# libav/libav

Hardware: AMD Instinct MI355X
Metric: macroblocks_per_s (higher is better)
Workload: dtype u8

## Files before the change

### include/mi355_h264_frame.h

```cpp
#ifndef MI355_H264_FRAME_H
#define MI355_H264_FRAME_H

#include <stddef.h>
#include <stdint.h>

#ifdef __cplusplus
extern "C" {
#endif

#define MI355_MB_INTRA4x4    0x00000001u
#define MI355_MB_INTRA16x16  0x00000002u
#define MI355_MB_INTRA_PCM   0x00000004u
#define MI355_MB_16x16       0x00000008u
#define MI355_MB_16x8        0x00000010u
#define MI355_MB_8x16        0x00000020u
#define MI355_MB_8x8         0x00000040u
#define MI355_MB_P0L0        0x00001000u
#define MI355_MB_P1L0        0x00002000u
#define MI355_MB_P0L1        0x00004000u
#define MI355_MB_P1L1        0x00008000u
#define MI355_MB_8x8DCT      0x01000000u
#define MI355_MB_INTRA       (MI355_MB_INTRA4x4 | MI355_MB_INTRA16x16 | MI355_MB_INTRA_PCM)

#define MI355_MBF_LEFT_EDGE  0x01
// ... 58 lines not shown
#define MI355_H264_MAX_SLOTS 32

typedef struct mi355_h264_slice {
    uint8_t use_weight;
    uint8_t use_weight_chroma;
    uint8_t luma_log2_weight_denom;
    uint8_t chroma_log2_weight_denom;
    uint8_t list_count;
    uint8_t reserved[3];
    uint8_t ref_slot[2][MI355_H264_MAX_REFS];
    int16_t luma_weight[MI355_H264_MAX_REFS][2][2];
    int16_t chroma_weight[MI355_H264_MAX_REFS][2][2][2];
    int16_t implicit_weight[MI355_H264_MAX_REFS][MI355_H264_MAX_REFS];
    uint8_t chroma_qp_table[2][52];
    int16_t implicit_weight_field[2][2 * MI355_H264_MAX_REFS][2 * MI355_H264_MAX_REFS];
} mi355_h264_slice;

typedef struct mi355_h264_frame {
    int32_t mb_width, mb_height;
    uint8_t *dst[3];
    int32_t dst_stride[2];
    uint8_t *recon[3];
    int32_t recon_stride[2];
    const uint8_t *ref[MI355_H264_MAX_SLOTS][3];
    const mi355_h264_mb *mb;
    const int16_t *mv[2];
    const int16_t *coef;
    const mi355_h264_slice *slices;
    int32_t nslices;
    int32_t max_intra_level;
    const uint32_t *intra_list;
    const int32_t *intra_level_start;
    int32_t max_level_width;
    int32_t field_picture;
    int32_t surface_layout;
    int32_t flags;
} mi355_h264_frame;
#define MI355_FRAME_NO_INTER 1
#define MI355_FRAME_MBAFF    2

#define MI355_SURFACE_LINEAR 0
#define MI355_SURFACE_TILED  1
#define MI355_LAYOUTS_LINEAR 1
#define MI355_LAYOUTS_TILED  2
#define MI355_TILE_LUMA_BYTES   256
#define MI355_TILE_CHROMA_BYTES 128

typedef struct mi355_surface_job {
    uint8_t *lin[3];
    uint8_t *tiled[2];
    int32_t lin_stride[2];
    int32_t tiled_stride[2];
    int32_t mb_width, mb_height;
    int32_t to_tiled;
    int32_t reserved0;
} mi355_surface_job;
int mi355_h264_surface_convert_dev(const mi355_surface_job *jobs, int n, int max_mb_width, int max_mb_height, void *stream);

int mi355_h264_decode_frames(const mi355_h264_frame *frames, int nframes, void *stream);

int mi355_h264_decode_frames_dev(const mi355_h264_frame *d_frames, int nframes,
                                 int max_mb_width, int max_mb_height, int max_intra_level,
                                 int max_level_width, void *stream);

int mi355_h264_decode_frames_levels_dev(const mi355_h264_frame *d_frames, int nframes,
                                        int max_mb_width, int max_mb_height, int max_intra_level,
                                        const int32_t *level_widths, void *stream);

int mi355_h264_decode_frames_layouts_dev(const mi355_h264_frame *d_frames, int nframes,
                                         int max_mb_width, int max_mb_height, int max_intra_level,
                                         const int32_t *level_widths, int layouts, void *stream);

int mi355_h264_decode_frames_wide_dev(const mi355_h264_frame *d_frames, int nframes, int max_mb_width, int max_mb_height,
                                      int max_intra_level, const int32_t *level_widths, int bit_depth, int chroma_format_idc,
                                      int passes, void *stream);

int mi355_h264_recon_intra_levels_dev(const mi355_h264_frame *d_frames, int nframes, int max_intra_level, const int32_t *level_widths, void *stream);
int mi355_h264_recon_intra_all_dev(const mi355_h264_frame *d_frames, int nframes, int max_mb_width, int max_mb_height, int max_intra_level, const int32_t *level_widths, void *stream);
int mi355_h264_recon_intra_plan(int max_mb_width, int max_mb_height, int max_intra_level, const int32_t *level_widths, int pinned, int *single, long long *per_picture);
int mi355_h264_recon_inter_dev(const mi355_h264_frame *d_frames, int nframes, int max_mb_width, int max_mb_height, void *stream);
int mi355_h264_recon_inter_layouts_dev(const mi355_h264_frame *d_frames, int nframes, int max_mb_width, int max_mb_height, int layouts, void *stream);
int mi355_h264_recon_run_plan(int nframes, int max_mb_width, int max_mb_height, int forced, int *run, int *runs_row);
int mi355_h264_recon_inter_run_dev(const mi355_h264_frame *d_frames, int nframes, int max_mb_width, int max_mb_height, int run, void *stream);
int mi355_h264_recon_inter_sparse_dev(const mi355_h264_frame *d_frames, int nframes, int max_mb_width, int max_mb_height, void *stream);
int mi355_h264_recon_intra_dev(const mi355_h264_frame *d_frames, int nframes, int max_intra_level, int max_level_width, void *stream);
int mi355_h264_deblock_dev(const mi355_h264_frame *d_frames, int nframes, int max_mb_width, int max_mb_height, void *stream);
int mi355_h264_deblock_layouts_dev(const mi355_h264_frame *d_frames, int nframes, int max_mb_width, int max_mb_height, int layouts, void *stream);
int mi355_h264_deblock_resident_dev(const mi355_h264_frame *d_frames, int nframes, int max_mb_width, int max_mb_height, int layouts,
                                    int resident_waves, void *stream);
int mi355_h264_deblock_resident(int nframes, int max_mb_width, int max_mb_height, int layouts, int cus, int shares, int *resident_waves);

typedef struct mi355_h264_deblock_plan_info {
    int32_t tiled_waves;
    int32_t linear_bands;
    int32_t skip_tiled;
    int32_t linear_launches;
} mi355_h264_deblock_plan_info;
int mi355_h264_deblock_plan(int nframes, int max_mb_width, int max_mb_height, int layouts, int cus, mi355_h264_deblock_plan_info *plan);
int mi355_h264_deblock_form_dev(const mi355_h264_frame *d_frames, int nframes, int max_mb_width, int max_mb_height, int layouts,
                                int tiled_waves, int linear_bands, void *stream);

int mi355_h264_intra_schedule(mi355_h264_mb *mb, int mb_width, int mb_height,
                              uint32_t *list, int32_t *level_start, int *max_level_width);

int mi355_h264_intra_schedule_mbaff(mi355_h264_mb *mb, int mb_width, int mb_height,
                                    uint32_t *list, int32_t *level_start, int *max_level_width);

void *mi355_malloc(size_t bytes);
void  mi355_free(void *dptr);
int   mi355_memcpy_h2d(void *dst, const void *src, size_t bytes);
int   mi355_memcpy_d2h(void *dst, const void *src, size_t bytes);
int   mi355_memcpy_d2d(void *dst, const void *src, size_t bytes);
int   mi355_sync(void *stream);
void  mi355_prefer_blocking_sync(int on);
void *mi355_host_alloc(size_t bytes);
void  mi355_host_free(void *p);
int   mi355_memcpy_h2d_async(void *dst, const void *src, size_t bytes, void *stream);
int   mi355_memcpy_d2h_async(void *dst, const void *src, size_t bytes, void *stream);
int   mi355_memcpy2d_d2h_async(void *dst, size_t dst_pitch, const void *src, size_t src_pitch, size_t width_bytes, size_t rows, void *stream);
int   mi355_memcpy2d_d2d_async(void *dst, size_t dst_pitch, const void *src, size_t src_pitch, size_t width_bytes, size_t rows, void *stream);
int   mi355_event_sync(void *event);
typedef struct mi355_copy_job {
    const void *src;
    void *dst;
    uint64_t bytes;
} mi355_copy_job;
int   mi355_copy_batch_dev(const mi355_copy_job *jobs, int n, size_t max_bytes, void *stream);
typedef struct mi355_h264_pipelines mi355_h264_pipelines;
mi355_h264_pipelines *mi355_h264_pipelines_create(int shares, int turns);
void mi355_h264_pipelines_destroy(mi355_h264_pipelines *p);
int  mi355_h264_pipelines_decode_dev(mi355_h264_pipelines *p, const mi355_h264_frame *d_frames, int nframes, int max_mb_width, int max_mb_height,
                                     int max_intra_level, const int32_t *level_widths, int layouts);
int  mi355_h264_pipelines_sync(mi355_h264_pipelines *p);
int  mi355_h264_pipelines_share(const mi355_h264_pipelines *p, int nframes, int share, int *first, int *count);
void mi355_h264_pipelines_timing(mi355_h264_pipelines *p, int on);
void mi355_h264_pipelines_join(mi355_h264_pipelines *p, int mode);
int  mi355_h264_pipelines_collect(mi355_h264_pipelines *p, double sums[3], int *launches);

void *mi355_stream_create(void);
void  mi355_stream_destroy(void *stream);
int   mi355_stream_wait_event(void *stream, void *event);
void *mi355_event_create(void);
void  mi355_event_destroy(void *event);
int   mi355_event_record(void *event, void *stream);
int   mi355_event_query(void *event);
float mi355_event_elapsed_ms(void *start, void *end);

#ifdef __cplusplus
}
#endif
#endif
```

### libav_amd/csrc/h264_frame.hip

```cpp
#include <cstdlib>
#include <vector>
#include "h264_recon_dev.h"
#include "../../include/mi355dsp.h"


namespace {

__attribute__((amdgpu_waves_per_eu(MI355_RECON_WAVES, MI355_RECON_WAVES)))
__global__ void __launch_bounds__(64)
k_recon_inter(const mi355_h264_frame *__restrict__ frames, int max_w, int max_h, unsigned long long inv_w, unsigned long long inv_h, int nblocks, int per_xcd)
{
    __shared__ MbLds s;
    recon_inter_wave<false>(s, frames, max_w, max_h, inv_w, inv_h, nblocks, per_xcd);
}
__attribute__((amdgpu_waves_per_eu(MI355_RECON_WAVES, MI355_RECON_WAVES)))
__global__ void __launch_bounds__(64)
k_recon_inter_sparse(const mi355_h264_frame *__restrict__ frames, int max_w, int max_h, unsigned long long inv_w, unsigned long long inv_h, int nblocks, int per_xcd)
{
    __shared__ MbLds s;
    recon_inter_wave<true>(s, frames, max_w, max_h, inv_w, inv_h, nblocks, per_xcd);
}

constexpr int TP = 32;
constexpr int CP = 16;
// ... 133 lines not shown
            MI355_WAVE_SYNC();
        }
    } else {
        for (int i = 0; i < 16; i++) {
            const int x0 = 4 * blk_x4(i), y0 = 4 * blk_y4(i);
            const int tr_ok = (h.topright_samples_available << i) & 0x8000;
            if (lane < 5) s.ps.T[lane] = TILE(x0 + lane - 1, y0 - 1);
            else if (lane < 9) s.ps.T[lane] = tr_ok ? TILE(x0 + lane - 1, y0 - 1) : TILE(x0 + 3, y0 - 1);
            if (lane >= 32 && lane < 37) s.ps.L[lane - 32] = TILE(x0 - 1, y0 + lane - 33);
            MI355_WAVE_SYNC();
            intra_pred_wave(s.ps, 0, h.u.intra4x4_pred_mode[i], 0, 0, &TILE(x0, y0), TP);
            const int q = lane & 3;
            int c[4], r[4], row;
#pragma unroll
            for (int k2 = 0; k2 < 4; k2++) c[k2] = s.mb.coef[i * 16 + q + 4 * k2];
            idct4_quad(c, q, r, row);
            if (lane < 4 && ((h.nnz_mask >> i) & 1)) add_row4<true>(&TILE(x0, y0 + row), r);
            MI355_WAVE_SYNC();
        }
    }
    if (!(t & MI355_MB_INTRA16x16)) residual_chroma<true>(s.mb, &CTILE(0, 0, 0), &CTILE(1, 0, 0), CP);
    intra_store_mb<TILED, AGENT>(&TILE(0, 0), TP, &CTILE(0, 0, 0), &CTILE(1, 0, 0), CP, fr, mb_x, mb_y);
}
#undef TILE

__global__ void __launch_bounds__(64)
k_recon_intra(const mi355_h264_frame *frames, int level, int width)
{
    __shared__ IntraLds s;
    const int f = blockIdx.x / width, k = blockIdx.x - f * width;
    const mi355_h264_frame &frd = frames[f];
    if (level > frd.max_intra_level) return;
    const int first = mi355_global(frd.intra_level_start)[level - 1], count = mi355_global(frd.intra_level_start)[level] - first;
    if (k >= count) return;
    const int mb_xy = (int)mi355_global(frd.intra_list)[first + k];
    if (uniform(frd.surface_layout) == MI355_SURFACE_TILED) recon_intra_mb<true>(s, frd, mb_xy);
    else recon_intra_mb<false>(s, frd, mb_xy);
}

constexpr int INTRA_SINGLE_LEVELS = 16;
constexpr uint32_t INTRA_NAPS_MAX = 1u << 21;
#ifdef MI355_HIP_EMU_H
static inline uint32_t intra_flag_word(const uint8_t *p) { uint32_t v; std::memcpy(&v, reinterpret_cast<const uint8_t *>(reinterpret_cast<uintptr_t>(p) & ~(uintptr_t)3), 4); return v; }
static inline void intra_flag_set(uint8_t *p) { *p = 1; }
#else
__device__ __forceinline__ uint32_t intra_flag_word(const uint8_t *p) { return agent_load_u32(reinterpret_cast<const uint32_t *>(reinterpret_cast<uintptr_t>(p) & ~(uintptr_t)3)); }
__device__ __forceinline__ void intra_flag_set(uint8_t *p) { __hip_atomic_store(p, (uint8_t)1, __ATOMIC_RELAXED, __HIP_MEMORY_SCOPE_AGENT); }
#endif
__global__ void __launch_bounds__(64)
k_recon_intra_all(const mi355_h264_frame *__restrict__ frames, int nframes, int nmb_max, uint8_t *__restrict__ flags, uint32_t *error_word, uint32_t naps_max)
{
    __shared__ IntraLds s;
    const int k = (int)(blockIdx.x / (unsigned)nframes), f = (int)(blockIdx.x - (unsigned)k * (unsigned)nframes);
    const mi355_h264_frame &frd = frames[f];
    const int nlev = uniform(frd.max_intra_level);
    if (nlev <= 0) return;
    if (k >= uniform(mi355_global(frd.intra_level_start)[nlev])) return;
    const int mb_xy = (int)uniform((int)mi355_global(frd.intra_list)[k]);
    const int W = uniform(frd.mb_width), mb_y = mb_xy / W, mb_x = mb_xy - mb_y * W;
    uint8_t *const pic_flags = mi355_global(flags) + (size_t)f * (size_t)nmb_max;
    const int lane = lane_id();
    const int nx = mb_x + (lane == 3 ? 1 : (lane == 2 ? 0 : -1)), ny = mb_y - (lane == 0 ? 0 : 1);
    const bool inside = lane < 4 && nx >= 0 && nx < W && ny >= 0;
    const int nxy = inside ? ny * W + nx : mb_xy;
    const bool dep = inside && (mi355_global_v(reinterpret_cast<const uint32_t *>(mi355_global(frd.mb) + nxy))[0] & MI355_MB_INTRA) != 0;
    static_assert(offsetof(mi355_h264_mb, mb_type) == 0, "the type word of a record");
    const bool waits = __any(dep);
    if (waits) {
        const uint8_t *fp = pic_flags + nxy;
        const int sh = 8 * (int)(reinterpret_cast<uintptr_t>(fp) & 3);
        uint32_t naps = 0;
        while (__any(dep && ((intra_flag_word(fp) >> sh) & 0xFFu) == 0) && naps < naps_max) { wave_nap(); naps++; }
        if (naps >= naps_max && __any(dep && ((intra_flag_word(fp) >> sh) & 0xFFu) == 0) && lane_id() == 0) atomicOr(error_word, (uint32_t)MI355_ERR_WAIT_EXPIRED);
        MI355_ISSUE_FENCE();
    }
    if (uniform(frd.surface_layout) == MI355_SURFACE_TILED) recon_intra_mb<true, true>(s, frd, mb_xy, waits);
    else recon_intra_mb<false, true>(s, frd, mb_xy, waits);
    agent_drain_stores();
    if (lane == 0 && naps_max) intra_flag_set(pic_flags + mb_xy);
}

}

static int recon_inter_launch(const mi355_h264_frame *d_frames, int nframes, int max_mb_width, int max_mb_height, bool sparse, void *stream, int layouts = MI355_LAYOUTS_LINEAR | MI355_LAYOUTS_TILED, int tiled_run = 0)
{
    if (!mi355::bind() || !d_frames || nframes <= 0) return -1;
    const int per_frame = max_mb_width * max_mb_height;
    if (per_frame <= 0 || per_frame >= (1 << 24)) return -3;
    const int frames_per_launch = ((1 << 24) - 1) / per_frame;
    const unsigned long long one = 1ull << 40;
    for (int f0 = 0; f0 < nframes; f0 += frames_per_launch) {
        const int nf = nframes - f0 < frames_per_launch ? nframes - f0 : frames_per_launch;
        const int nblocks = nf * per_frame, per_xcd = (nblocks + 7) / 8;
        const unsigned long long iw = (one + max_mb_width - 1) / max_mb_width, ih = (one + max_mb_height - 1) / max_mb_height;
        if (sparse)
            hipLaunchKernelGGL(k_recon_inter_sparse, dim3((unsigned)(8 * per_xcd)), dim3(64), 0, (hipStream_t)stream,
                               d_frames + f0, max_mb_width, max_mb_height, iw, ih, nblocks, per_xcd);
        else if (layouts == MI355_LAYOUTS_TILED) {
            if (!mi355::recon_inter_tiled_launch(d_frames + f0, nf, max_mb_width, max_mb_height, (hipStream_t)stream, tiled_run)) return -4;
        }
        else
            hipLaunchKernelGGL(k_recon_inter, dim3((unsigned)(8 * per_xcd)), dim3(64), 0, (hipStream_t)stream,
                               d_frames + f0, max_mb_width, max_mb_height, iw, ih, nblocks, per_xcd);
    }
    return hipGetLastError() == hipSuccess ? 0 : -2;
}
extern "C" int mi355_h264_recon_inter_dev(const mi355_h264_frame *d_frames, int nframes, int max_mb_width, int max_mb_height, void *stream)
{
    return recon_inter_launch(d_frames, nframes, max_mb_width, max_mb_height, false, stream);
}
extern "C" int mi355_h264_recon_inter_layouts_dev(const mi355_h264_frame *d_frames, int nframes, int max_mb_width, int max_mb_height, int layouts, void *stream)
{
    if (!(layouts & (MI355_LAYOUTS_LINEAR | MI355_LAYOUTS_TILED))) return -1;
    return recon_inter_launch(d_frames, nframes, max_mb_width, max_mb_height, false, stream, layouts);
}
extern "C" int mi355_h264_recon_inter_run_dev(const mi355_h264_frame *d_frames, int nframes, int max_mb_width, int max_mb_height, int run, void *stream)
{
    int r, runs_row;
    if (run <= 0 || !mi355::recon_run_plan(nframes, max_mb_width, max_mb_height, run, &r, &runs_row)) return -1;
    return recon_inter_launch(d_frames, nframes, max_mb_width, max_mb_height, false, stream, MI355_LAYOUTS_TILED, run);
}
extern "C" int mi355_h264_recon_inter_sparse_dev(const mi355_h264_frame *d_frames, int nframes, int max_mb_width, int max_mb_height, void *stream)
{
    return recon_inter_launch(d_frames, nframes, max_mb_width, max_mb_height, true, stream);
}

extern "C" int mi355_h264_recon_intra_dev(const mi355_h264_frame *d_frames, int nframes, int max_intra_level, int max_level_width, void *stream)
{
    if (!mi355::bind() || !d_frames || nframes <= 0) return -1;
    if (max_intra_level <= 0 || max_level_width <= 0) return 0;
    for (int level = 1; level <= max_intra_level; level++)
        hipLaunchKernelGGL(k_recon_intra, dim3((unsigned)(nframes * max_level_width)), dim3(64), 0, (hipStream_t)stream,
                           d_frames, level, max_level_width);
    return hipGetLastError() == hipSuccess ? 0 : -2;
}

static bool recon_intra_plan(int max_mb_width, int max_mb_height, int max_intra_level, const int32_t *level_widths, int pinned, long long *per_picture)
{
    *per_picture = 0;
    if (pinned == 0 || (pinned != 1 && max_intra_level < INTRA_SINGLE_LEVELS)) return false;
    long long sum = 0;
    for (int level = 1; level <= max_intra_level; level++) sum += level_widths[level - 1] > 0 ? level_widths[level - 1] : 0;
    const long long nmb = (long long)max_mb_width * max_mb_height;
    *per_picture = sum > nmb ? nmb : sum;
    return true;
}
static int intra_single_pin()
{
    static const int single = std::getenv("MI355_INTRA_SINGLE") ? std::atoi(std::getenv("MI355_INTRA_SINGLE")) : -1;
    return single;
}
extern "C" int mi355_h264_recon_intra_plan(int max_mb_width, int max_mb_height, int max_intra_level, const int32_t *level_widths, int pinned, int *single, long long *per_picture)
{
    if (max_mb_width <= 0 || max_mb_height <= 0 || max_intra_level < 0 || (max_intra_level > 0 && !level_widths) || !single || !per_picture) return -1;
    *single = recon_intra_plan(max_mb_width, max_mb_height, max_intra_level, level_widths, pinned < 0 ? intra_single_pin() : pinned, per_picture) ? 1 : 0;
    return 0;
}

extern "C" int mi355_h264_recon_intra_all_dev(const mi355_h264_frame *d_frames, int nframes, int max_mb_width, int max_mb_height, int max_intra_level, const int32_t *level_widths, void *stream)
{
    if (!mi355::bind() || !d_frames || nframes <= 0 || max_mb_width <= 0 || max_mb_height <= 0 || (max_intra_level > 0 && !level_widths)) return -1;
    long long per_picture = 0;
    if (!recon_intra_plan(max_mb_width, max_mb_height, max_intra_level, level_widths, intra_single_pin(), &per_picture))
        return mi355_h264_recon_intra_levels_dev(d_frames, nframes, max_intra_level, level_widths, stream);
    if (per_picture <= 0) return 0;
    const long long nmb = (long long)max_mb_width * max_mb_height;
    if ((long long)nframes * per_picture > 0x7FFFFFFFLL || (long long)nframes * nmb > 0x7FFFFFFFLL) return -3;
    const size_t bytes = ((size_t)nframes * (size_t)nmb + 3) & ~(size_t)3;
    uint32_t *flags = mi355::sync_words((hipStream_t)stream, bytes / 4);
    if (!flags) return -4;
    MI355_TRY(hipMemsetAsync(flags, 0, bytes, (hipStream_t)stream), -4);
    uint32_t *err = mi355::error_word();
    if (!err) return -4;
    static const uint32_t naps_max = std::getenv("MI355_INTRA_NAPS_MAX") ? (uint32_t)std::strtoul(std::getenv("MI355_INTRA_NAPS_MAX"), nullptr, 0) : INTRA_NAPS_MAX;
    hipLaunchKernelGGL(k_recon_intra_all, dim3((unsigned)(nframes * per_picture)), dim3(64), 0, (hipStream_t)stream, d_frames, nframes, (int)nmb, reinterpret_cast<uint8_t *>(flags), err, naps_max);
    return hipGetLastError() == hipSuccess ? 0 : -2;
}

extern "C" int mi355_h264_recon_intra_levels_dev(const mi355_h264_frame *d_frames, int nframes, int max_intra_level, const int32_t *level_widths, void *stream)
{
    if (!mi355::bind() || !d_frames || nframes <= 0 || (max_intra_level > 0 && !level_widths)) return -1;
    for (int level = 1; level <= max_intra_level; level++) {
        const int width = level_widths[level - 1];
        if (width <= 0) continue;
        if ((long long)nframes * width > 0x7FFFFFFFLL) return -3;
        hipLaunchKernelGGL(k_recon_intra, dim3((unsigned)(nframes * width)), dim3(64), 0, (hipStream_t)stream, d_frames, level, width);
    }
    return hipGetLastError() == hipSuccess ? 0 : -2;
}

#ifdef MI355_PROF
extern "C" void mi355_debug_rprof(unsigned long long *out, int reset)
{
    unsigned long long z[16] = {};
    MI355_CHECK(hipDeviceSynchronize());
    MI355_CHECK(hipMemcpyFromSymbol(out, HIP_SYMBOL(g_rprof), sizeof(z)));
    if (reset) MI355_CHECK(hipMemcpyToSymbol(HIP_SYMBOL(g_rprof), z, sizeof(z)));
}
#endif

extern "C" int mi355_h264_decode_frames_dev(const mi355_h264_frame *d_frames, int nframes, int max_mb_width, int max_mb_height,
                                            int max_intra_level, int max_level_width, void *stream)
{
// ... 279 lines not shown
```

### libav_amd/csrc/h264_frame_dev.h

```cpp
#ifndef MI355_H264_FRAME_DEV_H
#define MI355_H264_FRAME_DEV_H

#include "mi355_rt.h"
#include "h264_dev.h"
#include "../../include/mi355_h264_frame.h"

namespace mi355 {

typedef uint32_t mi355_u32x4 __attribute__((vector_size(16)));
typedef uint32_t mi355_u32x2 __attribute__((vector_size(8)));
typedef uint32_t mi355_u32x4u __attribute__((vector_size(16), aligned(4)));
typedef uint32_t mi355_u32x2u __attribute__((vector_size(8), aligned(4)));

__device__ __forceinline__ int blk_x4(int i) { return (i & 1) + 2 * ((i >> 2) & 1); }
__device__ __forceinline__ int blk_y4(int i) { return ((i >> 1) & 1) + 2 * (i >> 3); }
__device__ __forceinline__ int blk_index(int x4, int y4) { return (x4 & 1) + 2 * (y4 & 1) + 4 * (x4 >> 1) + 8 * (y4 >> 1); }

__device__ __forceinline__ uint32_t tile_y_off(int mb_x, int mb_y, int stride) { return (uint32_t)(__mul24(mb_y, stride) + mb_x * MI355_TILE_LUMA_BYTES); }
__device__ __forceinline__ uint32_t tile_c_off(int mb_x, int mb_y, int stride) { return (uint32_t)(__mul24(mb_y, stride) + mb_x * MI355_TILE_CHROMA_BYTES); }

__device__ __forceinline__ uint4 lds16(const uint8_t *p)
{
    const uint2 a = reinterpret_cast<const uint2 *>(p)[0], b = reinterpret_cast<const uint2 *>(p)[1];
    return make_uint4(a.x, a.y, b.x, b.y);
}
__device__ __forceinline__ void lds16(uint8_t *p, uint4 v)
{
    reinterpret_cast<mi355_u32x2 *>(p)[0] = mi355_u32x2{ v.x, v.y };
    reinterpret_cast<mi355_u32x2 *>(p)[1] = mi355_u32x2{ v.z, v.w };
}
__device__ __forceinline__ uint4 ld16(const uint8_t *p, bool al)
{
    if (al) return *reinterpret_cast<const uint4 *>(p);
    const uint32_t *w = reinterpret_cast<const uint32_t *>(p);
    return make_uint4(w[0], w[1], w[2], w[3]);
}
__device__ __forceinline__ void st16(uint8_t *p, uint4 v, bool al)
{
    if (al) { *reinterpret_cast<mi355_u32x4 *>(p) = mi355_u32x4{ v.x, v.y, v.z, v.w }; return; }
    uint32_t *w = reinterpret_cast<uint32_t *>(p);
    w[0] = v.x; w[1] = v.y; w[2] = v.z; w[3] = v.w;
}
__device__ __forceinline__ uint2 ld8(const uint8_t *p, bool al)
{
    if (al) return *reinterpret_cast<const uint2 *>(p);
    const uint32_t *w = reinterpret_cast<const uint32_t *>(p);
    return make_uint2(w[0], w[1]);
}
__device__ __forceinline__ void st8(uint8_t *p, uint2 v, bool al)
{
    if (al) { *reinterpret_cast<mi355_u32x2 *>(p) = mi355_u32x2{ v.x, v.y }; return; }
    uint32_t *w = reinterpret_cast<uint32_t *>(p);
    w[0] = v.x; w[1] = v.y;
}

bool recon_run_plan(int nframes, int max_w, int max_h, int forced, int *run, int *runs_row);
bool recon_inter_tiled_launch(const mi355_h264_frame *d_frames, int nframes, int max_w, int max_h, hipStream_t stream, int forced_run = 0);
void recon_inter_rest_launch(const mi355_h264_frame *d_frames, int max_w, int max_h, int run, int runs_row, unsigned long long inv_runs, unsigned long long inv_h, int nruns,
                             const uint32_t *rest, hipStream_t stream);
uint32_t *sync_words(hipStream_t stream, size_t words);
}
namespace {
#ifdef MI355_HIP_EMU_H
static inline uint32_t agent_load_u32(const uint32_t *p) { return *p; }
static inline void agent_store_u32(uint32_t *p, uint32_t v) { *p = v; }
static inline void agent_store8(uint8_t *p, uint2 v, bool al8) { mi355::st8(p, v, al8); }
static inline void agent_drain_stores() {}
static inline void wave_nap() { std::fprintf(stderr, "k_deblock_tiled: a band waits for a band that has not run (emulator: workgroups run in order)\n"); std::abort(); }
#else
__device__ __forceinline__ uint32_t agent_load_u32(const uint32_t *p) { return __hip_atomic_load(p, __ATOMIC_RELAXED, __HIP_MEMORY_SCOPE_AGENT); }
__device__ __forceinline__ void agent_store_u32(uint32_t *p, uint32_t v) { __hip_atomic_store(p, v, __ATOMIC_RELAXED, __HIP_MEMORY_SCOPE_AGENT); }
__device__ __forceinline__ void agent_store8(uint8_t *p, uint2 v, bool al8)
{
    if (al8) { __hip_atomic_store(reinterpret_cast<unsigned long long *>(p), (unsigned long long)v.x | ((unsigned long long)v.y << 32), __ATOMIC_RELAXED, __HIP_MEMORY_SCOPE_AGENT); return; }
    uint32_t *w = reinterpret_cast<uint32_t *>(p);
    agent_store_u32(w, v.x); agent_store_u32(w + 1, v.y);
}
__device__ __forceinline__ void agent_drain_stores() { asm volatile("s_waitcnt vmcnt(0)" ::: "memory"); }
__device__ __forceinline__ void wave_nap() { __builtin_amdgcn_s_sleep(16); }
#endif
}
#ifdef MI355_HIP_EMU_H
template <bool AGENT> static inline void lds_dma16(const uint8_t *src, uint8_t *lds_base) { std::memcpy(lds_base + 16 * (threadIdx.x & 63), src, 16); }
#else
template <bool AGENT> __device__ __forceinline__ void lds_dma16(const uint8_t *src, uint8_t *lds_base)
{
    typedef __attribute__((address_space(1))) const void *gptr;
    typedef __attribute__((address_space(3))) void *lptr;
    __builtin_amdgcn_global_load_lds((gptr)src, (lptr)lds_base, 16, 0, AGENT ? 16 : 0);
}
#endif
#ifdef MI355_HIP_EMU_H
static inline void lds_dma_wait() {}
#else
__device__ __forceinline__ void lds_dma_wait() { asm volatile("s_waitcnt vmcnt(0)" ::: "memory"); }
#endif

#endif
```

### libav_amd/csrc/h264_frame_tiled.hip

```cpp
#define MI355_PLAIN_LANE 1
#include "h264_recon_fast.h"

#include <cstdlib>

namespace {
__attribute__((amdgpu_waves_per_eu(MI355_RECON_WAVES, MI355_RECON_WAVES)))
__global__ void __launch_bounds__(64)
k_recon_inter_tiled(const mi355_h264_frame *__restrict__ frames, int max_w, int max_h, int run, int runs_row, unsigned long long inv_runs, unsigned long long inv_h, int nwaves, int per_xcd,
                    uint32_t *__restrict__ rest)
{
    __shared__ MbLds s;
    recon_inter_run(s, frames, max_w, max_h, run, runs_row, inv_runs, inv_h, nwaves, per_xcd, rest);
}
}

namespace mi355 {
bool recon_run_plan(int nframes, int max_w, int max_h, int forced, int *run_out, int *runs_row_out)
{
    if (nframes <= 0 || max_w <= 0 || max_h <= 0 || forced < 0) return false;
    const long long mbs = (long long)nframes * max_w * max_h;
    int run = (int)(mbs / (40ll * 8192));
    run = forced > 0 ? forced : (run < 4 ? 4 : (run > 15 ? 15 : run));
    if (run > max_w) run = max_w;
    const int runs_row = (max_w + run - 1) / run;
    run = (max_w + runs_row - 1) / runs_row;
    if (run > 16) return false;
    *run_out = run;
    *runs_row_out = runs_row;
    return true;
}

bool recon_inter_tiled_launch(const mi355_h264_frame *d_frames, int nframes, int max_w, int max_h, hipStream_t stream, int forced_run)
{
    static const int env = std::getenv("MI355_RECON_RUN") ? std::atoi(std::getenv("MI355_RECON_RUN")) : 0;
    static const int forced = env > 0 ? (env < 4 ? 4 : (env > 15 ? 15 : env)) : 0;
    int run, runs_row;
    if (!recon_run_plan(nframes, max_w, max_h, forced_run > 0 ? forced_run : forced, &run, &runs_row)) return false;
    const unsigned long long one = 1ull << 40;
    const long long total = (long long)nframes * max_h * runs_row;
    const int nwaves = (int)total, per_xcd = (nwaves + 7) / 8;
    uint32_t *rest = sync_words(stream, (size_t)nwaves);
    if (!rest) return false;
    const unsigned long long inv_runs = (one + runs_row - 1) / runs_row, inv_h = (one + max_h - 1) / max_h;
    hipLaunchKernelGGL(k_recon_inter_tiled, dim3((unsigned)(8 * per_xcd)), dim3(64), 0, stream, d_frames, max_w, max_h, run, runs_row, inv_runs, inv_h, nwaves, per_xcd, rest);
    recon_inter_rest_launch(d_frames, max_w, max_h, run, runs_row, inv_runs, inv_h, nwaves, rest, stream);
    return true;
}
}

extern "C" int mi355_h264_recon_run_plan(int nframes, int max_mb_width, int max_mb_height, int forced, int *run, int *runs_row)
{
    if (!run || !runs_row) return -1;
    return mi355::recon_run_plan(nframes, max_mb_width, max_mb_height, forced, run, runs_row) ? 0 : -1;
}
```

### libav_amd/csrc/h264_recon_fast.h

```cpp
#ifndef MI355_H264_RECON_FAST_H
#define MI355_H264_RECON_FAST_H

#include "h264_recon_dev.h"

namespace {

#if defined(FQ_MARKS) && !defined(MI355_HIP_EMU_H)
#define FQ_MARK(name) asm volatile("; MARK " name)
#else
#define FQ_MARK(name)
#endif

constexpr int FQ_COEF = (int)offsetof(MbCore, coef);
constexpr int FQ_RS = FQ_COEF + 768;
constexpr int FQ_RSC = FQ_RS + 512;
constexpr int FQ_ST = FQ_RS;
constexpr int FQ_WY = FQ_RS + 768;
constexpr int FQ_WC = FQ_WY + 1024;
constexpr int FQ_PL = FQ_WC + 256;
constexpr int FQ_PLANE = 16 * 24 + 8;
constexpr int FQ_DUMP = FQ_PL + 16 * 24;
constexpr int FQ_WSTEP = FQ_PL + 2 * FQ_PLANE - FQ_WY;
static_assert(FQ_RS == MB_PY_OFF && (FQ_WY % 16) == 0 && (FQ_PL % 8) == 0 && (FQ_WSTEP % 16) == 0 && FQ_WC + FQ_WSTEP + 256 <= (int)sizeof(MbLds), "fast-path regions inside MbLds");
static_assert(FQ_WY + FQ_WSTEP + 48 * 20 + 24 + 16 + 12 <= (int)sizeof(MbLds), "the second half of a transposing product reads window rows 16..20");
// ... 421 lines not shown
    uint8_t *const base = reinterpret_cast<uint8_t *>(&s);
    FQ_MARK("luma_resid");
    if (has_resid) {
        const mi355_u32x2 r = *reinterpret_cast<const mi355_u32x2 *>(base + k.rsy);
        const uint32_t s01 = pk_sat_u8(pk_add(byte_perm(0u, v, 0x0C010C00u), r[0])), s23 = pk_sat_u8(pk_add(byte_perm(0u, v, 0x0C030C02u), r[1]));
        v = byte_perm(s23, s01, 0x05040100u);
    }
    MI355_WAVE_SYNC();
    *reinterpret_cast<uint32_t *>(base + FQ_ST + k.sy) = v;
}
__device__ __forceinline__ void fq_luma(MbLds &s, const FqLane &k, int so2, int pos, bool has_resid) { fq_luma_out(s, k, fq_luma_pred(s, k, so2, pos), has_resid); }

__device__ __forceinline__ uint32_t fq_chroma_pred(MbLds &s, const FqLane &k, int oc, uint32_t wts)
{
    uint8_t *const base = reinterpret_cast<uint8_t *>(&s);
    const uint32_t at = k.c1 + (uint32_t)oc, sh = at & 3u;
    const uint32_t r0 = fq_bytes4(base + (at & ~3u), sh), r1 = fq_bytes4(base + (at & ~3u) + 12, sh);
    const uint32_t d0 = fq_dot4(byte_perm(r1, r0, 0x05040100u), wts, 32u), d1 = fq_dot4(byte_perm(r1, r0, 0x06050201u), wts, 32u);
    return (d0 >> 6) | ((d1 >> 6) << 8);
}
__device__ __forceinline__ void fq_chroma_out(MbLds &s, const FqLane &k, uint32_t two, bool has_resid)
{
    uint8_t *const base = reinterpret_cast<uint8_t *>(&s);
    if (has_resid) two = pk_sat_u8(pk_add(byte_perm(0u, two, 0x0C010C00u), *reinterpret_cast<const uint32_t *>(base + k.rsc)));
    *reinterpret_cast<uint16_t *>(base + FQ_ST + 256 + k.sc) = (uint16_t)two;
}
__device__ __forceinline__ void fq_chroma(MbLds &s, const FqLane &k, int oc, uint32_t wts, bool has_resid) { fq_chroma_out(s, k, fq_chroma_pred(s, k, oc, wts), has_resid); }
__device__ __forceinline__ void fq_store(MbLds &s, uint8_t *ytile, uint8_t *ctile)
{
    const uint8_t *const base = reinterpret_cast<const uint8_t *>(&s);
    const int lane = lane_id();
    if (lane < 24) {
        const mi355_u32x4 v = *reinterpret_cast<const mi355_u32x4 *>(base + FQ_ST + 16 * lane);
        if (lane < 16) *reinterpret_cast<mi355_u32x4 *>(ytile + (uint32_t)(16 * lane)) = v;
        else *reinterpret_cast<mi355_u32x4 *>(ctile + (uint32_t)(16 * lane - 256)) = v;
    }
}

__device__ __forceinline__ void fq_two(MbLds &s, const FqLane &k, const ResidLane &rl, const FqPic &pic, int mb_xy, int mb_x, int mb_y)
{
    fq_kptr h = fq_konst(pic.mb + mb_xy), mv = fq_konst(pic.mv0 + (size_t)mb_xy * 32);
    const uint32_t type = h[0], nnz = h[1], w2 = h[2], w12 = h[12], w14 = h[14];
    const bool vsplit = (type & MI355_MB_8x16) != 0, has_chroma = (w2 & 0x30u) != 0, resid = (nnz & 0xFFFFu) != 0 || has_chroma;
    const int woff = 0;
    const int n1 = vsplit ? 2 : 8, q1 = vsplit ? 8 : 16;
    const FqGeo g0 = fq_geometry(mv[0], mb_x, mb_y, (int8_t)(w14 & 0xFFu), w12 & 0xFFu, pic.hot.mb_width, pic.hot.mb_height);
    const FqGeo g1 = fq_geometry(mv[n1], mb_x, mb_y, (int8_t)((w14 >> q1) & 0xFFu), (w12 >> q1) & 0xFFu, pic.hot.mb_width, pic.hot.mb_height);
    const int set0 = woff, set1 = woff ^ FQ_WSTEP;
    auto issue = [&](const FqGeo &g, int set) {
        const uint64_t need = fq_need(g.a);
        if (g.a & FQA_INSIDE) fq_windows_issue_inside(s, k, pic.desc, pic.hot, (int)((g.a >> 17) & 31u), (int16_t)(g.d & 0xFFFFu), (int16_t)(g.e & 0xFFFFu), (int)g.d >> 16, (int)g.e >> 16, set, need);
        else fq_windows_issue(s, k, pic.desc, pic.hot, (int)((g.a >> 17) & 31u), (int16_t)(g.d & 0xFFFFu), (int16_t)(g.e & 0xFFFFu), (int)g.d >> 16, (int)g.e >> 16, set, need);
    };
    issue(g0, set0);
    issue(g1, set1);
    if (resid) fq_coef_dma(s, k, pic.coef, mb_xy);
    fq_wait_vm0();
    MI355_WAVE_SYNC();
    if (resid) fq_idct(s, k, rl, nnz, has_chroma, pic.mb + mb_xy);
    if ((g0.a | g1.a) & (FQA_PATCH_Y | FQA_PATCH_C)) {
        fq_windows_patch(s, k, (g0.a & FQA_PATCH_Y) != 0, (g0.a & FQA_PATCH_C) != 0, (int16_t)(g0.e & 0xFFFFu), (int)g0.e >> 16, set0, pic.hot.mb_width, fq_need(g0.a));
        fq_windows_patch(s, k, (g1.a & FQA_PATCH_Y) != 0, (g1.a & FQA_PATCH_C) != 0, (int16_t)(g1.e & 0xFFFFu), (int)g1.e >> 16, set1, pic.hot.mb_width, fq_need(g1.a));
    }
    MI355_WAVE_SYNC();
    const int lane = lane_id();
    const bool second_y = vsplit ? lane >= 32 : (lane & 8) != 0, second_c = vsplit ? (lane & 2) != 0 : (lane & 16) != 0;
    uint32_t vy = 0, vc = 0;
#pragma nounroll
    for (int p = 0; p < 2; p++) {
        const uint32_t ga = p ? g1.a : g0.a, gw = p ? g1.wts : g0.wts;
        const int set = p ? set1 : set0;
        const uint32_t y = fq_luma_pred(s, k, (int)(ga & 31u) + set, (int)((ga >> 7) & 15u));
        const uint32_t c = fq_chroma_pred(s, k, (int)((ga >> 5) & 3u) + set, gw);
        if (second_y == (p != 0)) vy = y;
        if (second_c == (p != 0)) vc = c;
    }
    fq_luma_out(s, k, vy, resid);
    fq_chroma_out(s, k, vc, resid);
    MI355_WAVE_SYNC();
    fq_store(s, pic.hot.recon[0] + tile_y_off(mb_x, mb_y, pic.hot.recon_stride[0]), pic.hot.recon[1] + tile_c_off(mb_x, mb_y, pic.hot.recon_stride[1]));
    MI355_WAVE_SYNC();
}

__device__ __forceinline__ void recon_inter_run(MbLds &s, const mi355_h264_frame *__restrict__ frames, int max_w, int max_h, int run, int runs_row,
                                                unsigned long long inv_runs, unsigned long long inv_h, int nwaves, int per_xcd, uint32_t *__restrict__ rest)
{
    const int wave = xcd_linear((int)blockIdx.x, per_xcd);
    if (wave >= nwaves) return;
    const int row = div_magic(wave, inv_runs);
    const int mb_x = (wave - row * runs_row) * run;
    const int f = div_magic(row, inv_h), mb_y = row - f * max_h;
    const int n = max_w - mb_x < run ? max_w - mb_x : run;
    ResidLane rl;
    resid_lane_compute(rl);
    const FqLane k = fq_lane();
    auto picture = [&](int pf, FqPic &pic) -> bool {
        const mi355_h264_frame &frd = frames[pf];
        pic.hot = frame_hot(frd);
        pic.mb = pic.hot.mb; pic.mv0 = pic.hot.mv[0]; pic.coef = pic.hot.coef; pic.desc = &frd;
        return uniform(frd.surface_layout) == MI355_SURFACE_TILED && !(uniform(frd.flags) & MI355_FRAME_NO_INTER);
    };
    FqPic pic;
    const bool pic_ok = picture(f, pic);
    const int n_row = pic_ok && mb_x < pic.hot.mb_width && mb_y < pic.hot.mb_height ? (n < pic.hot.mb_width - mb_x ? n : pic.hot.mb_width - mb_x) : 0;
    uint32_t deferred = 0;
    if (n_row > 0) {
        const int mb_xy0 = mb_y * pic.hot.mb_width + mb_x;
        const FqRun run = fq_describe(pic, mb_xy0, mb_x, mb_y, n_row);
        uint32_t ra = run.a, rw = run.wts, rn = run.nnz, rd = run.d, re = run.e;
        MI355_PIN(ra); MI355_PIN(rw); MI355_PIN(rn); MI355_PIN(rd); MI355_PIN(re);
        bool pre_w = false, pre_c = false;
        uint32_t a = fq_lane_word(ra, 0);
        for (int i = 0; i < n_row; i++) {
            const bool has_next = i + 1 < n_row;
            const uint32_t an = has_next ? fq_lane_word(ra, i + 1) : 0u;
            const int woff = (i & 1) * FQ_WSTEP;
            bool next_w = false, next_c = false;
            if (a & FQA_FAST) {
                auto issue = [&](int m, uint32_t am, int set) {
                    const uint32_t d = fq_lane_word(rd, m), e = fq_lane_word(re, m);
                    const uint64_t need = fq_need(am);
                    if (am & FQA_INSIDE) fq_windows_issue_inside(s, k, pic.desc, pic.hot, (int)((am >> 17) & 31u), (int16_t)(d & 0xFFFFu), (int16_t)(e & 0xFFFFu), (int)d >> 16, (int)e >> 16, set, need);
                    else fq_windows_issue(s, k, pic.desc, pic.hot, (int)((am >> 17) & 31u), (int16_t)(d & 0xFFFFu), (int16_t)(e & 0xFFFFu), (int)d >> 16, (int)e >> 16, set, need);
                };
                FQ_MARK("issue");
                if (!pre_w) issue(i, a, woff);
                if ((a & FQA_RESID) && !pre_c) fq_coef_dma(s, k, pic.coef, mb_xy0 + i);
                next_w = (an & FQA_FAST) != 0;
                if (next_w) issue(i + 1, an, woff ^ FQ_WSTEP);
                if (next_w) fq_wait_vm2(); else fq_wait_vm0();
                MI355_WAVE_SYNC();
                FQ_MARK("idct");
                if (a & FQA_RESID) fq_idct(s, k, rl, fq_lane_word(rn, i), (a & FQA_CHROMA) != 0, pic.mb + (mb_xy0 + i));
                MI355_WAVE_SYNC();
                FQ_MARK("coefnext");
                next_c = next_w && (an & FQA_RESID);
                if (next_c) fq_coef_dma(s, k, pic.coef, mb_xy0 + i + 1);
                if (a & (FQA_PATCH_Y | FQA_PATCH_C)) {
                    const uint32_t e = fq_lane_word(re, i);
                    fq_windows_patch(s, k, (a & FQA_PATCH_Y) != 0, (a & FQA_PATCH_C) != 0, (int16_t)(e & 0xFFFFu), (int)e >> 16, woff, pic.hot.mb_width, fq_need(a));
                    MI355_WAVE_SYNC();
                }
                FQ_MARK("luma");
                fq_luma(s, k, (int)(a & 31u) + woff, (int)((a >> 7) & 15u), (a & FQA_RESID) != 0);
                FQ_MARK("chroma");
                fq_chroma(s, k, (int)((a >> 5) & 3u) + woff, fq_lane_word(rw, i), (a & FQA_RESID) != 0);
                MI355_WAVE_SYNC();
                FQ_MARK("store");
                fq_store(s, pic.hot.recon[0] + tile_y_off(mb_x + i, mb_y, pic.hot.recon_stride[0]), pic.hot.recon[1] + tile_c_off(mb_x + i, mb_y, pic.hot.recon_stride[1]));
                MI355_WAVE_SYNC();
            } else if (!(a & FQA_INTRA)) {
                deferred |= (a & FQA_TWO) ? 0x10000u << i : 1u << i;
            }
            FQ_MARK("tail");
            pre_w = next_w; pre_c = next_c;
            a = an;
        }
    }
    if (lane_id() == 0) rest[wave] = deferred;
}

constexpr int FQ_REST = 8;
__device__ __forceinline__ void recon_inter_rest(MbLds &s, const mi355_h264_frame *__restrict__ frames, int max_w, int max_h, int run, int runs_row,
                                                 unsigned long long inv_runs, unsigned long long inv_h, int nruns, int ngroups, int per_xcd, const uint32_t *__restrict__ rest)
{
    const int g = xcd_linear((int)blockIdx.x, per_xcd);
    if (g >= ngroups) return;
    const int r = FQ_REST * g + (lane_id() & (FQ_REST - 1));
    const uint32_t mine = r < nruns ? rest[r] : 0u;
    if (!__any(mine != 0)) return;
    auto place = [&](int j, int &f, int &mb_x, int &mb_y) {
        const int w = FQ_REST * g + j;
        const int row = div_magic(w, inv_runs);
        mb_x = (w - row * runs_row) * run;
        f = div_magic(row, inv_h); mb_y = row - f * max_h;
    };
    if (__any((mine >> 16) != 0)) {
        ResidLane rl;
        resid_lane_compute(rl);
        const FqLane k = fq_lane();
        for (int j = 0; j < FQ_REST; j++) {
            uint32_t m = fq_lane_word(mine, j) >> 16;
            if (!m) continue;
            int f, mb_x, mb_y;
            place(j, f, mb_x, mb_y);
            const mi355_h264_frame &frd = frames[f];
            if (uniform(frd.surface_layout) != MI355_SURFACE_TILED) continue;
            FqPic pic;
            pic.hot = frame_hot(frd);
            pic.mb = pic.hot.mb; pic.mv0 = pic.hot.mv[0]; pic.coef = pic.hot.coef; pic.desc = &frd;
            while (m) {
                const int i = __builtin_ctz(m);
                m &= m - 1;
                fq_two(s, k, rl, pic, mb_y * pic.hot.mb_width + mb_x + i, mb_x + i, mb_y);
                fq_wait_vm0();
                MI355_WAVE_SYNC();
            }
        }
    }
    for (int j = 0; j < FQ_REST; j++) {
        uint32_t m = fq_lane_word(mine, j) & 0xFFFFu;
        if (!m) continue;
        int f, mb_x, mb_y;
        place(j, f, mb_x, mb_y);
        if (uniform(frames[f].surface_layout) != MI355_SURFACE_TILED) continue;
        while (m) {
            const int i = __builtin_ctz(m);
            m &= m - 1;
            recon_inter_mb<false, true>(s, frames[f], mb_x + i, mb_y);
            fq_wait_vm0();
            MI355_WAVE_SYNC();
        }
    }
}

}
#endif
```

Before: 1.515 billion.

## Let one tiled inter-recon wave cover a span of several macroblock runs

Adds a span parameter so each wave in the tiled inter-reconstruction kernel processes several consecutive runs of a row instead of one. It also adds a planner and API to choose the span, and writes the per-run deferred masks with a lane-parallel ballot instead of accumulating them in a loop. The aim is fewer waves and less per-wave setup on large workloads, at the cost of less parallelism. Because RECON_SPAN_MAX is 1, the automatic plan always picks span 1, so default behaviour changes only through the new deferred-word bookkeeping.

After: 1.507 billion. About the same (-0.5%).

```diff
diff --git a/include/mi355_h264_frame.h b/include/mi355_h264_frame.h
--- a/include/mi355_h264_frame.h
+++ b/include/mi355_h264_frame.h
@@ -164,6 +164,8 @@
 int mi355_h264_recon_inter_layouts_dev(const mi355_h264_frame *d_frames, int nframes, int max_mb_width, int max_mb_height, int layouts, void *stream);
 int mi355_h264_recon_run_plan(int nframes, int max_mb_width, int max_mb_height, int forced, int *run, int *runs_row);
 int mi355_h264_recon_inter_run_dev(const mi355_h264_frame *d_frames, int nframes, int max_mb_width, int max_mb_height, int run, void *stream);
+int mi355_h264_recon_span_plan(int nframes, int max_mb_width, int max_mb_height, int forced_run, int forced_span, int *run, int *runs_row, int *span);
+int mi355_h264_recon_inter_span_dev(const mi355_h264_frame *d_frames, int nframes, int max_mb_width, int max_mb_height, int run, int span, void *stream);
 int mi355_h264_recon_inter_sparse_dev(const mi355_h264_frame *d_frames, int nframes, int max_mb_width, int max_mb_height, void *stream);
 int mi355_h264_recon_intra_dev(const mi355_h264_frame *d_frames, int nframes, int max_intra_level, int max_level_width, void *stream);
 int mi355_h264_deblock_dev(const mi355_h264_frame *d_frames, int nframes, int max_mb_width, int max_mb_height, void *stream);
diff --git a/libav_amd/csrc/h264_frame.hip b/libav_amd/csrc/h264_frame.hip
--- a/libav_amd/csrc/h264_frame.hip
+++ b/libav_amd/csrc/h264_frame.hip
@@ -239,7 +239,7 @@
 
 }
 
-static int recon_inter_launch(const mi355_h264_frame *d_frames, int nframes, int max_mb_width, int max_mb_height, bool sparse, void *stream, int layouts = MI355_LAYOUTS_LINEAR | MI355_LAYOUTS_TILED, int tiled_run = 0)
+static int recon_inter_launch(const mi355_h264_frame *d_frames, int nframes, int max_mb_width, int max_mb_height, bool sparse, void *stream, int layouts = MI355_LAYOUTS_LINEAR | MI355_LAYOUTS_TILED, int tiled_run = 0, int tiled_span = 0)
 {
     if (!mi355::bind() || !d_frames || nframes <= 0) return -1;
     const int per_frame = max_mb_width * max_mb_height;
@@ -254,7 +254,7 @@
             hipLaunchKernelGGL(k_recon_inter_sparse, dim3((unsigned)(8 * per_xcd)), dim3(64), 0, (hipStream_t)stream,
                                d_frames + f0, max_mb_width, max_mb_height, iw, ih, nblocks, per_xcd);
         else if (layouts == MI355_LAYOUTS_TILED) {
-            if (!mi355::recon_inter_tiled_launch(d_frames + f0, nf, max_mb_width, max_mb_height, (hipStream_t)stream, tiled_run)) return -4;
+            if (!mi355::recon_inter_tiled_launch(d_frames + f0, nf, max_mb_width, max_mb_height, (hipStream_t)stream, tiled_run, tiled_span)) return -4;
         }
         else
             hipLaunchKernelGGL(k_recon_inter, dim3((unsigned)(8 * per_xcd)), dim3(64), 0, (hipStream_t)stream,
@@ -275,7 +275,13 @@
 {
     int r, runs_row;
     if (run <= 0 || !mi355::recon_run_plan(nframes, max_mb_width, max_mb_height, run, &r, &runs_row)) return -1;
-    return recon_inter_launch(d_frames, nframes, max_mb_width, max_mb_height, false, stream, MI355_LAYOUTS_TILED, run);
+    return recon_inter_launch(d_frames, nframes, max_mb_width, max_mb_height, false, stream, MI355_LAYOUTS_TILED, run, 1);
+}
+extern "C" int mi355_h264_recon_inter_span_dev(const mi355_h264_frame *d_frames, int nframes, int max_mb_width, int max_mb_height, int run, int span, void *stream)
+{
+    int r, runs_row, sp;
+    if (run <= 0 || span <= 0 || !mi355::recon_span_plan(nframes, max_mb_width, max_mb_height, run, span, &r, &runs_row, &sp)) return -1;
+    return recon_inter_launch(d_frames, nframes, max_mb_width, max_mb_height, false, stream, MI355_LAYOUTS_TILED, run, span);
 }
 extern "C" int mi355_h264_recon_inter_sparse_dev(const mi355_h264_frame *d_frames, int nframes, int max_mb_width, int max_mb_height, void *stream)
 {
diff --git a/libav_amd/csrc/h264_frame_dev.h b/libav_amd/csrc/h264_frame_dev.h
--- a/libav_amd/csrc/h264_frame_dev.h
+++ b/libav_amd/csrc/h264_frame_dev.h
@@ -55,7 +55,8 @@
 }
 
 bool recon_run_plan(int nframes, int max_w, int max_h, int forced, int *run, int *runs_row);
-bool recon_inter_tiled_launch(const mi355_h264_frame *d_frames, int nframes, int max_w, int max_h, hipStream_t stream, int forced_run = 0);
+bool recon_span_plan(int nframes, int max_w, int max_h, int forced_run, int forced_span, int *run, int *runs_row, int *span);
+bool recon_inter_tiled_launch(const mi355_h264_frame *d_frames, int nframes, int max_w, int max_h, hipStream_t stream, int forced_run = 0, int forced_span = 0);
 void recon_inter_rest_launch(const mi355_h264_frame *d_frames, int max_w, int max_h, int run, int runs_row, unsigned long long inv_runs, unsigned long long inv_h, int nruns,
                              const uint32_t *rest, hipStream_t stream);
 uint32_t *sync_words(hipStream_t stream, size_t words);
diff --git a/libav_amd/csrc/h264_frame_tiled.hip b/libav_amd/csrc/h264_frame_tiled.hip
--- a/libav_amd/csrc/h264_frame_tiled.hip
+++ b/libav_amd/csrc/h264_frame_tiled.hip
@@ -6,11 +6,11 @@
 namespace {
 __attribute__((amdgpu_waves_per_eu(MI355_RECON_WAVES, MI355_RECON_WAVES)))
 __global__ void __launch_bounds__(64)
-k_recon_inter_tiled(const mi355_h264_frame *__restrict__ frames, int max_w, int max_h, int run, int runs_row, unsigned long long inv_runs, unsigned long long inv_h, int nwaves, int per_xcd,
-                    uint32_t *__restrict__ rest)
+k_recon_inter_tiled(const mi355_h264_frame *__restrict__ frames, int max_w, int max_h, int run, int runs_row, int span, int spans_row, unsigned long long inv_spans, unsigned long long inv_h,
+                    int nwaves, int per_xcd, uint32_t *__restrict__ rest)
 {
     __shared__ MbLds s;
-    recon_inter_run(s, frames, max_w, max_h, run, runs_row, inv_runs, inv_h, nwaves, per_xcd, rest);
+    recon_inter_run(s, frames, max_w, max_h, run, runs_row, span, spans_row, inv_spans, inv_h, nwaves, per_xcd, rest);
 }
 }
 
@@ -30,20 +30,47 @@
     return true;
 }
 
-bool recon_inter_tiled_launch(const mi355_h264_frame *d_frames, int nframes, int max_w, int max_h, hipStream_t stream, int forced_run)
+constexpr int RECON_RUN_LONG = 15, RECON_SPAN_MAX = 1, RECON_SPAN_ROUNDS = 10;
+bool recon_span_plan(int nframes, int max_w, int max_h, int forced_run, int forced_span, int *run_out, int *runs_row_out, int *span_out)
+{
+    int run, runs_row;
+    if (forced_span < 0 || !recon_run_plan(nframes, max_w, max_h, forced_run, &run, &runs_row)) return false;
+    int span = 1;
+    if (forced_span > 0) {
+        if (forced_span * run > 64) return false;
+        span = forced_span;
+    } else if ((long long)nframes * max_w * max_h / (40ll * 8192) >= RECON_RUN_LONG) {
+        const long long rows = (long long)nframes * max_h;
+        for (int s = 2; s <= RECON_SPAN_MAX && s * run <= 64 && s <= runs_row; s++)
+            if (rows * ((runs_row + s - 1) / s) >= (long long)RECON_SPAN_ROUNDS * 8192) span = s;
+    }
+    *run_out = run;
+    *runs_row_out = runs_row;
+    *span_out = span;
+    return true;
+}
+
+bool recon_inter_tiled_launch(const mi355_h264_frame *d_frames, int nframes, int max_w, int max_h, hipStream_t stream, int forced_run, int forced_span)
 {
     static const int env = std::getenv("MI355_RECON_RUN") ? std::atoi(std::getenv("MI355_RECON_RUN")) : 0;
     static const int forced = env > 0 ? (env < 4 ? 4 : (env > 15 ? 15 : env)) : 0;
-    int run, runs_row;
-    if (!recon_run_plan(nframes, max_w, max_h, forced_run > 0 ? forced_run : forced, &run, &runs_row)) return false;
+    static const int env_span = std::getenv("MI355_RECON_SPAN") ? std::atoi(std::getenv("MI355_RECON_SPAN")) : 0;
+    int run, runs_row, span;
+    if (forced_span > 0 || env_span <= 0) {
+        if (!recon_span_plan(nframes, max_w, max_h, forced_run > 0 ? forced_run : forced, forced_span, &run, &runs_row, &span)) return false;
+    } else {
+        if (!recon_span_plan(nframes, max_w, max_h, forced_run > 0 ? forced_run : forced, 1, &run, &runs_row, &span)) return false;
+        span = env_span < 64 / run ? env_span : 64 / run;
+    }
     const unsigned long long one = 1ull << 40;
-    const long long total = (long long)nframes * max_h * runs_row;
-    const int nwaves = (int)total, per_xcd = (nwaves + 7) / 8;
-    uint32_t *rest = sync_words(stream, (size_t)nwaves);
+    const int spans_row = (runs_row + span - 1) / span;
+    const long long rows = (long long)nframes * max_h;
+    const int nruns = (int)(rows * runs_row), nwaves = (int)(rows * spans_row), per_xcd = (nwaves + 7) / 8;
+    uint32_t *rest = sync_words(stream, (size_t)nruns);
     if (!rest) return false;
-    const unsigned long long inv_runs = (one + runs_row - 1) / runs_row, inv_h = (one + max_h - 1) / max_h;
-    hipLaunchKernelGGL(k_recon_inter_tiled, dim3((unsigned)(8 * per_xcd)), dim3(64), 0, stream, d_frames, max_w, max_h, run, runs_row, inv_runs, inv_h, nwaves, per_xcd, rest);
-    recon_inter_rest_launch(d_frames, max_w, max_h, run, runs_row, inv_runs, inv_h, nwaves, rest, stream);
+    const unsigned long long inv_runs = (one + runs_row - 1) / runs_row, inv_spans = (one + spans_row - 1) / spans_row, inv_h = (one + max_h - 1) / max_h;
+    hipLaunchKernelGGL(k_recon_inter_tiled, dim3((unsigned)(8 * per_xcd)), dim3(64), 0, stream, d_frames, max_w, max_h, run, runs_row, span, spans_row, inv_spans, inv_h, nwaves, per_xcd, rest);
+    recon_inter_rest_launch(d_frames, max_w, max_h, run, runs_row, inv_runs, inv_h, nruns, rest, stream);
     return true;
 }
 }
@@ -53,3 +80,9 @@
     if (!run || !runs_row) return -1;
     return mi355::recon_run_plan(nframes, max_mb_width, max_mb_height, forced, run, runs_row) ? 0 : -1;
 }
+
+extern "C" int mi355_h264_recon_span_plan(int nframes, int max_mb_width, int max_mb_height, int forced_run, int forced_span, int *run, int *runs_row, int *span)
+{
+    if (!run || !runs_row || !span) return -1;
+    return mi355::recon_span_plan(nframes, max_mb_width, max_mb_height, forced_run, forced_span, run, runs_row, span) ? 0 : -1;
+}
diff --git a/libav_amd/csrc/h264_recon_fast.h b/libav_amd/csrc/h264_recon_fast.h
--- a/libav_amd/csrc/h264_recon_fast.h
+++ b/libav_amd/csrc/h264_recon_fast.h
@@ -527,15 +527,17 @@
     MI355_WAVE_SYNC();
 }
 
-__device__ __forceinline__ void recon_inter_run(MbLds &s, const mi355_h264_frame *__restrict__ frames, int max_w, int max_h, int run, int runs_row,
-                                                unsigned long long inv_runs, unsigned long long inv_h, int nwaves, int per_xcd, uint32_t *__restrict__ rest)
+__device__ __forceinline__ void recon_inter_run(MbLds &s, const mi355_h264_frame *__restrict__ frames, int max_w, int max_h, int run, int runs_row, int span, int spans_row,
+                                                unsigned long long inv_spans, unsigned long long inv_h, int nwaves, int per_xcd, uint32_t *__restrict__ rest)
 {
     const int wave = xcd_linear((int)blockIdx.x, per_xcd);
     if (wave >= nwaves) return;
-    const int row = div_magic(wave, inv_runs);
-    const int mb_x = (wave - row * runs_row) * run;
+    const int row = div_magic(wave, inv_spans);
+    const int run0 = (wave - row * spans_row) * span;
+    const int nruns = runs_row - run0 < span ? runs_row - run0 : span;
+    const int mb_x = run0 * run;
     const int f = div_magic(row, inv_h), mb_y = row - f * max_h;
-    const int n = max_w - mb_x < run ? max_w - mb_x : run;
+    const int n = max_w - mb_x < span * run ? max_w - mb_x : span * run;
     ResidLane rl;
     resid_lane_compute(rl);
     const FqLane k = fq_lane();
@@ -548,13 +550,22 @@
     FqPic pic;
     const bool pic_ok = picture(f, pic);
     const int n_row = pic_ok && mb_x < pic.hot.mb_width && mb_y < pic.hot.mb_height ? (n < pic.hot.mb_width - mb_x ? n : pic.hot.mb_width - mb_x) : 0;
-    uint32_t deferred = 0;
+    auto put_words = [&](uint64_t general, uint64_t two) {
+        const int r = lane_id();
+        const uint32_t sh = (uint32_t)__mul24(r < nruns ? r : 0, run), m = (1u << run) - 1u;
+        if (r < nruns) rest[row * runs_row + run0 + r] = ((uint32_t)(general >> sh) & m) | (((uint32_t)(two >> sh) & m) << 16);
+    };
     if (n_row > 0) {
         const int mb_xy0 = mb_y * pic.hot.mb_width + mb_x;
-        const FqRun run = fq_describe(pic, mb_xy0, mb_x, mb_y, n_row);
-        uint32_t ra = run.a, rw = run.wts, rn = run.nnz, rd = run.d, re = run.e;
+        const FqRun dsc = fq_describe(pic, mb_xy0, mb_x, mb_y, n_row);
+        uint32_t ra = dsc.a, rw = dsc.wts, rn = dsc.nnz, rd = dsc.d, re = dsc.e;
         MI355_PIN(ra); MI355_PIN(rw); MI355_PIN(rn); MI355_PIN(rd); MI355_PIN(re);
         bool pre_w = false, pre_c = false;
+        {
+            const uint64_t live = n_row < 64 ? (1ull << n_row) - 1ull : ~0ull;
+            const bool left = !(ra & (FQA_FAST | FQA_INTRA));
+            put_words(lane_mask(left && !(ra & FQA_TWO)) & live, lane_mask(left && (ra & FQA_TWO)) & live);
+        }
         uint32_t a = fq_lane_word(ra, 0);
         for (int i = 0; i < n_row; i++) {
             const bool has_next = i + 1 < n_row;
@@ -594,15 +605,14 @@
                 FQ_MARK("store");
                 fq_store(s, pic.hot.recon[0] + tile_y_off(mb_x + i, mb_y, pic.hot.recon_stride[0]), pic.hot.recon[1] + tile_c_off(mb_x + i, mb_y, pic.hot.recon_stride[1]));
                 MI355_WAVE_SYNC();
-            } else if (!(a & FQA_INTRA)) {
-                deferred |= (a & FQA_TWO) ? 0x10000u << i : 1u << i;
             }
             FQ_MARK("tail");
             pre_w = next_w; pre_c = next_c;
             a = an;
         }
-    }
-    if (lane_id() == 0) rest[wave] = deferred;
+    } else {
+        put_words(0, 0);
+    }
 }
 
 constexpr int FQ_REST = 8;
```
